# alexandrainst/coral

Hardware: AMD Instinct MI355X
Metric: audio-seconds/sec (CTC finetune step: fwd+bwd+allreduce+clip+AdamW), wav2vec2-large, 10 s utterances (higher is better)
Workload: dtype bf16; 1 GPU; wav2vec2-large (XLS-R shape d=1920 L=48 ffn=7680) CTC finetune, 8 x 10 s per GPU, SpecAugment on, activation_dropout 0.1, layerdrop 0 (multi-GPU rule), fp32 master + AdamW + clip 1.0; global_batch=8, frames_per_utt=499, parallelism=dp1

## Files before the change

### coral_amd/_lib.py

```python

from __future__ import annotations

import ctypes as C
import os
from pathlib import Path

_HERE = Path(__file__).resolve().parent
LIB_PATH = _HERE / "libcoral_amd.so"


class CoralAmdError(RuntimeError):
    """Raised when the HIP library is missing or a call into it fails."""


class CaGemmDesc(C.Structure):

    _fields_ = [
        ("A", C.c_void_p),
        ("B", C.c_void_p),
        ("C", C.c_void_p),
        ("C2", C.c_void_p),
        ("R", C.c_void_p),
        ("bias", C.c_void_p),
        ("M", C.c_int32),
# ... 220 lines not shown
                               _vp]),
    "ca_beam_select_workspace_bytes": (_i64, [_i32, _i32, _i32]),
    "ca_beam_select": (C.c_int, [_vp, _i64, _vp, _vp, _i32, _i32, _i32, _vp, _vp, _vp, _vp, _i64, _vp]),
    "ca_beam_advance": (C.c_int, [C.POINTER(CaBeamDesc), _vp]),
    "ca_mask_frames": (C.c_int, [_vp, _vp, _vp, _vp, _vp, _i32, _i32, _i32, _vp]),
    "ca_regroup_pad": (C.c_int, [_vp, _vp, _i32, _i32, _i32, _i32, _i32, _vp]),
    "ca_posconv_partial_floats": (_i64, [_i32]),
    "ca_posconv_weight": (C.c_int, [_vp, _vp, _vp, _vp, _vp, _vp, _i32, _i32, _i32, _vp]),
    "ca_posconv_weight_bwd": (
        C.c_int,
        [_vp, _vp, _vp, _vp, _vp, _vp, _vp, _i32, _i32, _i32, _vp],
    ),
    "ca_cast_f32_bf16": (C.c_int, [_vp, _vp, _i64, _vp]),
    "ca_cast_bf16_f32": (C.c_int, [_vp, _vp, _i64, _vp]),
    "ca_transpose_f32_bf16": (C.c_int, [_vp, _vp, _i32, _i32, _vp]),
    "ca_conv_weight_reorder": (C.c_int, [_vp, _vp, _i32, _i32, _i32, _vp]),
    "ca_conv_weight_grad_reorder": (C.c_int, [_vp, _vp, _i32, _i32, _i32, _vp]),
    "ca_sumsq_f32": (C.c_int, [_vp, _i64, _vp, _i32, _vp, _vp]),
    "ca_sumsq_ranges_f32": (C.c_int, [_vp, _vp, _i32, _vp, _i32, _vp, _vp]),
    "ca_clear_ranges": (C.c_int, [_vp, _vp, _i32, _i64, _vp]),
    "ca_sum_f32": (C.c_int, [_vp, _i64, _vp, _i32, _vp, _vp]),
    "ca_adamw_step": (
        C.c_int,
        [_vp, _vp, _vp, _vp, _vp, _i64, _f32, _f32, _f32, _f32, _f32, _i32, _f32, _f32, _vp, _vp],
    ),
    "ca_adamw_step_ex": (
        C.c_int,
        [_vp, _vp, _vp, _vp, _vp, _i64, _f32, _f32, _f32, _f32, _f32, _i32, _f32, _f32, _vp, _i32, _vp],
    ),
    "ca_adamw_step_g16": (
        C.c_int,
        [_vp, _vp, _vp, _vp, _vp, _i64, _f32, _f32, _f32, _f32, _f32, _i32, _f32, _f32, _vp, _i32, _vp],
    ),
    "ca_logmel_workspace_bytes": (_i64, [_i32]),
    "ca_logmel": (C.c_int, [_vp, _vp, _vp, _vp, _i32, _i64, _i32, _vp]),
    "ca_cross_entropy_fwd_bwd": (
        C.c_int,
        [_vp, _vp, _vp, _vp, _vp, _i64, _i32, _i64, _i32, _vp],
    ),
    "ca_argmax_masked": (C.c_int, [_vp, _vp, _vp, _i64, _i32, _i64, _vp]),
    "ca_whisper_decode_token": (C.c_int, [C.POINTER(CaDecodeDesc), _vp]),
    "ca_whisper_decode_token_supported": (C.c_int, [_i32, _i32, _i32, _i32, _i32]),
    "ca_debug_decode_stamps": (C.c_int, [_vp, _i32]),
    "ca_argmax_advance": (C.c_int, [_vp, _vp, _vp, _i64, _i32, _i64, _vp, _vp, _i64, _vp, _vp, _vp, _i32, _i32, _vp]),
    "ca_argmax_timestamps": (C.c_int, [_vp, _vp, _vp, _i64, _i32, _i64, _vp, _i64, _vp, _i32, _i32, _i32, _i32, _vp]),
    "ca_argmax_timestamps_advance": (C.c_int, [_vp, _vp, _vp, _i64, _i32, _i64, _vp, _vp, _i64, _vp, _vp, _vp, _i32, _i32,
                                               _i32, _i32, _i32, _vp]),
    "ca_pick_scored_advance": (C.c_int, [_vp, _vp, _vp, _i64, _i32, _i64, _f32, _vp, _i64, _vp, _vp, _vp, _vp, _i64, _vp, _vp,
                                         _vp, _i32, _i32, _vp, _i32, _i32, _i32, _vp]),
    "ca_row_token_prob": (C.c_int, [_vp, _vp, _i64, _i32, _i64, _i32, _vp]),
    "ca_whisper_align_cost": (C.c_int, [_vp, C.POINTER(_vp), _i32, C.POINTER(_i32), _i32, _i32, _i32, _i32, _i32, _i32, _i64,
                                        _i64, _vp, _i32, _f32, _i32, _vp, _vp, _i64, _vp]),
    "ca_dtw_token_times": (C.c_int, [_vp, _i32, _i32, _vp, _i32, _vp, _vp, _vp, _vp, _vp, _vp]),
    "ca_embed_tokens": (C.c_int, [_vp, _vp, _vp, _vp, _vp, _i64, _i32, _vp]),
    "ca_embed_tokens_bwd": (C.c_int, [_vp, _vp, _vp, _vp, _vp, _i64, _i32, _vp]),
    "ca_comm_unique_id": (C.c_int, [_vp]),
    "ca_comm_init": (C.c_int, [C.POINTER(_vp), _vp, _i32, _i32]),
    "ca_comm_destroy": (C.c_int, [_vp]),
    "ca_comm_abort": (C.c_int, [_vp]),
    "ca_comm_stream": (_vp, [_vp]),
    "ca_comm_rank": (C.c_int, [_vp]),
    "ca_comm_world": (C.c_int, [_vp]),
    "ca_comm_after": (C.c_int, [_vp, _vp]),
    "ca_comm_before": (C.c_int, [_vp, _vp]),
    "ca_allreduce_bucket": (C.c_int, [_vp, _vp, _i64, _i32]),
    "ca_reduce_scatter_bucket": (C.c_int, [_vp, _vp, _i64, _i32]),
# ... 30 lines not shown
```

### coral_amd/csrc/misc.hip

```cpp
#include "common.h"
#include <cstdlib>

__global__ __launch_bounds__(256) void mask_frames_kernel(unsigned short* __restrict__ h,
                                                          const uint8_t* __restrict__ tmask,
                                                          const uint8_t* __restrict__ fmask,
                                                          const unsigned short* __restrict__ embed,
                                                          const int32_t* __restrict__ flen, int B,
                                                          int T, int C) {
  const int cch = C >> 3;
  const int64_t total = (int64_t)B * T * cch;
  for (int64_t i = (int64_t)blockIdx.x * 256 + threadIdx.x; i < total;
       i += (int64_t)gridDim.x * 256) {
    const int c8 = (int)(i % cch);
    const int64_t bt = i / cch;
    const int t = (int)(bt % T), b = (int)(bt / T);
    const bool tm = tmask && tmask[bt];
    const bool pad = flen && t >= flen[b];
    bool anyf = false;
    if (fmask) {
#pragma unroll
      for (int e = 0; e < 8; ++e) anyf |= fmask[(int64_t)b * C + c8 * 8 + e] != 0;
    }
    if (!tm && !pad && !anyf) continue;
    unsigned short* p = h + bt * C + c8 * 8;
// ... 472 lines not shown
    if (threadIdx.x == 0) partial[c] = red[0] + red[1] + red[2] + red[3];
  }
}
extern "C" int ca_sumsq_ranges_f32(const float* g, const int64_t* chunks, int32_t nchunks, float* out,
                                   int32_t accumulate, float* partial, void* stream) {
  CA_CHECK_ARG(g && chunks && out && partial && nchunks > 0, "ca_sumsq_ranges_f32: bad argument");
  CA_CHECK_ARG(((uintptr_t)g % 16) == 0, "ca_sumsq_ranges_f32: g must be 16-byte aligned");
  hipStream_t s = (hipStream_t)stream;
  const int grid = nchunks < 2048 ? nchunks : 2048;
  hipLaunchKernelGGL(sumsq_chunks_kernel, dim3(grid), dim3(256), 0, s, g, chunks, nchunks, partial);
  hipLaunchKernelGGL(sumsq_finish_kernel, dim3(1), dim3(256), 0, s, partial, nchunks, out, accumulate);
  CA_CHECK_LAUNCH("ca_sumsq_ranges_f32");
  return CA_OK;
}
__global__ __launch_bounds__(256) void sum_kernel(const float* __restrict__ x, int64_t n, float* __restrict__ partial) {
  __shared__ float red[4];
  float a = 0.f;
  for (int64_t i = (int64_t)blockIdx.x * 256 + threadIdx.x; i < n; i += (int64_t)gridDim.x * 256) a += x[i];
  a = wave_sum(a);
  if ((threadIdx.x & 63) == 0) red[threadIdx.x >> 6] = a;
  __syncthreads();
  if (threadIdx.x == 0) partial[blockIdx.x] = red[0] + red[1] + red[2] + red[3];
}
extern "C" int ca_sum_f32(const float* x, int64_t n, float* out, int32_t accumulate, float* partial, void* stream) {
  CA_CHECK_ARG(x && out && partial && n > 0, "ca_sum_f32: bad argument");
  hipStream_t s = (hipStream_t)stream;
  const int grid = (int)((n + 255) / 256 < 256 ? (n + 255) / 256 : 256);
  hipLaunchKernelGGL(sum_kernel, dim3(grid), dim3(256), 0, s, x, n, partial);
  hipLaunchKernelGGL(sumsq_finish_kernel, dim3(1), dim3(256), 0, s, partial, grid, out, accumulate);
  CA_CHECK_LAUNCH("ca_sum_f32");
  return CA_OK;
}

template <bool NT, bool G16 = false>
__global__ __launch_bounds__(256) void adamw_kernel(float* __restrict__ p, float* __restrict__ m,
                                                    float* __restrict__ v,
                                                    const void* __restrict__ gv,
                                                    unsigned short* __restrict__ p16, int64_t n,
                                                    float lr, float b1, float b2, float eps,
                                                    float wd, float bc1, float bc2_sqrt,
                                                    float grad_scale, float max_norm,
                                                    const float* __restrict__ gnorm_sq, int allow_vec) {
  float coef = grad_scale;
  if (gnorm_sq && max_norm > 0.f) {
    const float nrm = sqrtf(gnorm_sq[0]) * grad_scale;
    const float c = max_norm / (nrm + 1e-6f);
    coef *= c < 1.f ? c : 1.f;
  }
  const float step_size = lr / bc1;
  const float decay = 1.f - lr * wd;
  const float* g = (const float*)gv;
  const unsigned short* g16 = (const unsigned short*)gv;
  const bool vec = allow_vec && ((((uintptr_t)p | (uintptr_t)m | (uintptr_t)v | (G16 ? 0 : (uintptr_t)gv)) & 15) == 0) &&
                   (!G16 || ((uintptr_t)gv & 7) == 0) && (!p16 || ((uintptr_t)p16 & 7) == 0);
  const int64_t n4 = vec ? (n >> 2) : 0;
  for (int64_t i = (int64_t)blockIdx.x * 256 + threadIdx.x; i < n4; i += (int64_t)gridDim.x * 256) {
    f32x4_t g4;
    if constexpr (G16) {
      const u16x4_t h = NT ? __builtin_nontemporal_load((const u16x4_t*)g16 + i) : ((const u16x4_t*)g16)[i];
      g4 = (f32x4_t){bf2f(h[0]), bf2f(h[1]), bf2f(h[2]), bf2f(h[3])};
    } else {
      g4 = NT ? __builtin_nontemporal_load((const f32x4_t*)g + i) : ((const f32x4_t*)g)[i];
    }
    f32x4_t p4 = NT ? __builtin_nontemporal_load((const f32x4_t*)p + i) : ((const f32x4_t*)p)[i];
    f32x4_t m4 = NT ? __builtin_nontemporal_load((const f32x4_t*)m + i) : ((const f32x4_t*)m)[i];
    f32x4_t v4 = NT ? __builtin_nontemporal_load((const f32x4_t*)v + i) : ((const f32x4_t*)v)[i];
    u16x4_t h4;
#pragma unroll
    for (int e = 0; e < 4; ++e) {
      const float gi = g4[e] * coef;
      float pi = p4[e] * decay;
      const float mi = b1 * m4[e] + (1.f - b1) * gi;
      const float vi = b2 * v4[e] + (1.f - b2) * gi * gi;
      const float denom = sqrtf(vi) / bc2_sqrt + eps;
      pi -= step_size * mi / denom;
      p4[e] = pi;
      m4[e] = mi;
      v4[e] = vi;
      h4[e] = f2bf(pi);
    }
    if (NT) {
      __builtin_nontemporal_store(p4, (f32x4_t*)p + i);
      __builtin_nontemporal_store(m4, (f32x4_t*)m + i);
      __builtin_nontemporal_store(v4, (f32x4_t*)v + i);
    } else {
      ((f32x4_t*)p)[i] = p4;
      ((f32x4_t*)m)[i] = m4;
      ((f32x4_t*)v)[i] = v4;
    }
    if (p16) ((u16x4_t*)p16)[i] = h4;
  }
  for (int64_t i = n4 * 4 + (int64_t)blockIdx.x * 256 + threadIdx.x; i < n; i += (int64_t)gridDim.x * 256) {
    const float gi = (G16 ? bf2f(g16[i]) : g[i]) * coef;
    float pi = p[i] * decay;
    const float mi = b1 * m[i] + (1.f - b1) * gi;
    const float vi = b2 * v[i] + (1.f - b2) * gi * gi;
    const float denom = sqrtf(vi) / bc2_sqrt + eps;
    pi -= step_size * mi / denom;
    p[i] = pi;
    m[i] = mi;
    v[i] = vi;
    if (p16) p16[i] = f2bf(pi);
  }
}
static int adamw_launch(float* p, float* m, float* v, const void* g, bool g16, void* p16, int64_t n, float lr, float beta1,
                        float beta2, float eps, float weight_decay, int32_t step, float grad_scale, float max_norm,
                        const float* gnorm_sq, int32_t max_blocks, void* stream) {
  CA_CHECK_ARG(p && m && v && g && n > 0 && step >= 1 && max_blocks >= 0, "ca_adamw_step: bad argument");
  const float bc1 = 1.f - powf(beta1, (float)step);
  const float bc2 = 1.f - powf(beta2, (float)step);
  static const int cap_env = [] { const char* e = getenv("CA_ADAMW_BLOCKS"); return e ? atoi(e) : 0; }();
  static const int vec = [] { const char* e = getenv("CA_ADAMW_VEC"); return e ? atoi(e) : 1; }();
  static const int nt = [] { const char* e = getenv("CA_ADAMW_NT"); return e ? atoi(e) : 1; }();
  const int cap = cap_env > 0 ? cap_env : max_blocks;
  int grid = ew_grid(n, vec ? 4 : 1);
  if (cap > 0 && grid > cap) grid = cap;
#define ADAMW(NTV, G16V)                                                                                              \
  hipLaunchKernelGGL((adamw_kernel<NTV, G16V>), dim3(grid), dim3(256), 0, (hipStream_t)stream, p, m, v, g,            \
                     (unsigned short*)p16, n, lr, beta1, beta2, eps, weight_decay, bc1, sqrtf(bc2), grad_scale,       \
                     max_norm, gnorm_sq, vec)
  if (nt && g16) ADAMW(true, true);
  else if (nt) ADAMW(true, false);
  else if (g16) ADAMW(false, true);
  else ADAMW(false, false);
#undef ADAMW
  CA_CHECK_LAUNCH("ca_adamw_step");
  return CA_OK;
}
const void* ca_adamw_background_kernel() { return (const void*)adamw_kernel<true, true>; }
extern "C" int ca_adamw_step_ex(float* p, float* m, float* v, const float* g, void* p16, int64_t n,
                                float lr, float beta1, float beta2, float eps, float weight_decay,
                                int32_t step, float grad_scale, float max_norm,
                                const float* gnorm_sq, int32_t max_blocks, void* stream) {
  return adamw_launch(p, m, v, g, false, p16, n, lr, beta1, beta2, eps, weight_decay, step, grad_scale, max_norm, gnorm_sq,
                      max_blocks, stream);
}
extern "C" int ca_adamw_step_g16(float* p, float* m, float* v, const void* g_bf16, void* p16, int64_t n,
                                 float lr, float beta1, float beta2, float eps, float weight_decay,
                                 int32_t step, float grad_scale, float max_norm,
                                 const float* gnorm_sq, int32_t max_blocks, void* stream) {
  return adamw_launch(p, m, v, g_bf16, true, p16, n, lr, beta1, beta2, eps, weight_decay, step, grad_scale, max_norm,
                      gnorm_sq, max_blocks, stream);
}
extern "C" int ca_adamw_step(float* p, float* m, float* v, const float* g, void* p16, int64_t n,
                             float lr, float beta1, float beta2, float eps, float weight_decay,
                             int32_t step, float grad_scale, float max_norm,
                             const float* gnorm_sq, void* stream) {
  return ca_adamw_step_ex(p, m, v, g, p16, n, lr, beta1, beta2, eps, weight_decay, step, grad_scale, max_norm, gnorm_sq, 0,
                          stream);
}

__global__ __launch_bounds__(256) void embed_kernel(const unsigned short* __restrict__ table,
                                                    const unsigned short* __restrict__ pos,
                                                    const int32_t* __restrict__ ids,
                                                    const int32_t* __restrict__ pos_ids,
                                                    unsigned short* __restrict__ y, int64_t rows,
                                                    int C) {
  const int cch = C >> 3;
  const int64_t total = rows * cch;
  for (int64_t i = (int64_t)blockIdx.x * 256 + threadIdx.x; i < total;
       i += (int64_t)gridDim.x * 256) {
    const int c8 = (int)(i % cch);
// ... 56 lines not shown
```

### coral_amd/ops.py

```python

from __future__ import annotations

import ctypes as C
import os

import torch

from . import _lib
from ._lib import (CaAttnDesc, EPI_DGELU, EPI_GELU, EPI_GELU_RESIDUAL, EPI_NONE, EPI_RESIDUAL, KMAJOR,
                   MNMAJOR, CaGemmDesc, CoralAmdError, check)

__all__ = ["KMAJOR", "MNMAJOR", "EPI_NONE", "EPI_GELU", "EPI_RESIDUAL", "EPI_DGELU",
           "EPI_GELU_RESIDUAL", "CoralAmdError"]

_ELT = {torch.bfloat16: 2, torch.float32: 4, torch.int32: 4, torch.uint8: 1, torch.int64: 8, torch.int16: 2,
        torch.uint32: 4}


def _stream() -> int:
    return torch.cuda.current_stream().cuda_stream


def _p(t: torch.Tensor | None, off: int = 0) -> int | None:
    if t is None:
# ... 571 lines not shown
        if any(a % 4 or n % 4 for a, n in rows):
            raise CoralAmdError("clear_ranges: ranges must be multiples of 4 bytes")
        big = [r for r in rows if r[1] >= (1 << 20)]
        small = [r for r in rows if r[1] < (1 << 20)]
        ent = tuple((torch.tensor(part, dtype=torch.int64, device=x.device), len(part), max(n for _, n in part))
                    for part in (big, small) if part)
        _CLEAR_TABLES[key] = ent
    for table, count, longest in ent:
        check(lib().ca_clear_ranges(_p(x), _p(table), count, longest, _stream()), "ca_clear_ranges")


def sumsq(g, n, out, partial, accumulate=False):
    check(lib().ca_sumsq_f32(_p(g), n, _p(out), int(accumulate), _p(partial), _stream()),
          "ca_sumsq_f32")


def sumsq_ranges(g, chunks, nchunks, out, partial, accumulate=False):
    check(lib().ca_sumsq_ranges_f32(_p(g), _p(chunks), nchunks, _p(out), int(accumulate), _p(partial), _stream()),
          "ca_sumsq_ranges_f32")


def sum_f32(x, n, out, partial, accumulate=False):
    check(lib().ca_sum_f32(_p(x), n, _p(out), int(accumulate), _p(partial), _stream()), "ca_sum_f32")


def adamw_step(p, m, v, g, p16, n, lr, beta1, beta2, eps, weight_decay, step, grad_scale=1.0,
               max_norm=0.0, gnorm_sq=None, max_blocks=0):
    fn = lib().ca_adamw_step_g16 if g.dtype == torch.bfloat16 else lib().ca_adamw_step_ex
    check(fn(_p(p), _p(m), _p(v), _p(g), _p(p16), n, lr, beta1, beta2, eps,
             weight_decay, step, grad_scale, max_norm, _p(gnorm_sq), int(max_blocks), _stream()),
          "ca_adamw_step")


def logmel_workspace_bytes(B):
    return lib().ca_logmel_workspace_bytes(B)


def logmel(wave, mel_filters, out, ws, B, N, n_mels):
    check(lib().ca_logmel(_p(wave), _p(mel_filters), _p(out), _p(ws), B, N, n_mels, _stream()),
          "ca_logmel")


def cross_entropy_fwd_bwd(logits, labels, loss_sum, count, grad, rows, V, ldv, ignore_index=-100):
    check(lib().ca_cross_entropy_fwd_bwd(_p(logits), _p(labels), _p(loss_sum), _p(count), _p(grad),
                                         rows, V, ldv, ignore_index, _stream()),
          "ca_cross_entropy_fwd_bwd")


def argmax_masked(logits, suppress, out, rows, V, ldv):
    check(lib().ca_argmax_masked(_p(logits), _p(suppress), _p(out), rows, V, ldv, _stream()),
          "ca_argmax_masked")


def argmax_advance(logits, suppress, out, rows, V, ldv, done, ids, tok, pos, klen, pad_id, eos_id):
    if done.dtype != torch.bool or ids.dtype != torch.int64 or ids.dim() != 2 or ids.stride(1) != 1:
        raise CoralAmdError("argmax_advance: done must be bool, ids a row-major int64 matrix")
    check(lib().ca_argmax_advance(_p(logits), _p(suppress), _p(out), rows, V, ldv, done.data_ptr(), _p(ids), ids.stride(0),
                                  _p(tok), _p(pos), _p(klen), int(pad_id), int(eos_id), _stream()), "ca_argmax_advance")


def _cap(max_initial_timestamp_index):
    return -1 if max_initial_timestamp_index is None else int(max_initial_timestamp_index)


def argmax_timestamps(logits, suppress, out, rows, V, ldv, ids, pos, begin_index, timestamp_begin, eos_id,
                      max_initial_timestamp_index=None):
# ... 185 lines not shown
```

### coral_amd/trainer.py

```python

from __future__ import annotations

import logging
import math
import os
import warnings

import torch

from . import ops
from .exchange import GradSync, collectives_selfcheck


def cosine_lr(step: int, base_lr: float, warmup_steps: int, max_steps: int) -> float:
    if step < warmup_steps:
        return base_lr * step / max(1, warmup_steps)
    progress = (step - warmup_steps) / max(1, max_steps - warmup_steps)
    return base_lr * max(0.0, 0.5 * (1.0 + math.cos(math.pi * progress)))


def grad_accumulation_steps(total_batch_size: int, num_devices: int, per_device_batch_size: int) -> int:
    return max(1, total_batch_size // max(1, num_devices) // per_device_batch_size)


# ... 60 lines not shown
        self.grad_accum = grad_accum
        if accum_loss not in ("mean", "sum"):
            raise ValueError(f"accum_loss must be 'mean' or 'sum', not {accum_loss!r}")
        self.accum_loss = accum_loss
        self.opt_step = 0
        st = engine.store
        lo, hi = self.train_range = tuple(engine.trainable_range())
        whole = (lo, hi) == (0, st.numel)
        world = 1
        if torch.distributed.is_available() and torch.distributed.is_initialized():
            world = torch.distributed.get_world_size(process_group)
        zero_stage = int(os.environ.get("CA_ZERO_STAGE", zero_stage) or 0)
        shard = {}
        if zero_stage and (world > 1 or os.environ.get("CA_DP_FORCE", "0") == "1") and whole:
            shard = {n: r for n, r in engine.shard_ranges().items() if (r[1] - r[0]) % (8 * world) == 0 and r[1] > r[0]}
        self.sync = GradSync(st.g32, st.buckets, process_group, compress=compress_grads, shard=shard)
        self.zero = bool(shard) and self.sync.active
        if self.zero and world > 1 and st.p32.is_cuda and not collectives_selfcheck(st.device, process_group, self.sync.capi):
            logging.getLogger(__package__).warning("sharded optimiser: the collective self-check failed; using replicated DDP")
            self.sync.close(abort=True)
            self.sync = GradSync(st.g32, st.buckets, process_group, compress=compress_grads)
            self.zero = False
        self.world = self.sync.world
        self.dist = self.sync.active
        self._set_compute_cus = False
        if self.dist and st.p32.is_cuda:
            ncu = torch.cuda.get_device_properties(st.device).multi_processor_count
            ops.lib().ca_gemm_set_compute_cus(int(os.environ.get("CA_COMPUTE_CUS", ncu)))
            self._set_compute_cus = True
        self.overlap = overlap and self.dist
        self._layout = state_layout(st.buckets, self.sync.shard if self.zero else {}, self.sync.rank, self.world)
        self._launches = [split_bf16(self._layout, r) for r in ({}, {} if self.zero else engine.bf16_grad_ranges())]
        self._forward_order = sorted(st.buckets, key=lambda name: st.buckets[name][0])
        self.m = torch.zeros(state_size(self._layout), dtype=torch.float32, device=st.device)
        self.v = torch.zeros_like(self.m)
        self._ag_comm = self.sync.capi if self.zero else None
        self._ag_stream = None
        if self.zero and st.p32.is_cuda:
            self._ag_stream = self._ag_comm.stream if self._ag_comm is not None else ops.side_stream(st.device, "gather")
        self.gnorm_sq = torch.zeros(1, dtype=torch.float32, device=st.device)
        self.partial = torch.zeros(4096, dtype=torch.float32, device=st.device)
        self.overlap_optimizer = (overlap_optimizer and os.environ.get("CA_OPT_OVERLAP", "1") != "0"
                                  and st.p32.is_cuda and whole)
        self.opt_stream = None
        if self.overlap_optimizer:
            prio = int(os.environ.get("CA_OPT_PRIO", "0"))
            self.opt_stream = ops.side_stream(st.device, "optimizer", prio)
        self.opt_done = None
        self.bg_blocks = 0
        if self.overlap_optimizer:
            bg = os.environ.get("CA_OPT_BG_BLOCKS")
            self.bg_blocks = int(bg) if bg is not None else torch.cuda.get_device_properties(st.device).multi_processor_count
            if bg is None:
                fits, rx, ru = ops.background_update_fits()
                if not fits:
                    warnings.warn(f"coral_amd: the forward GEMM kernel holds {rx} registers per lane and the update "
                                  f"kernel {ru}: the update cannot run beside it; using the full-grid update")
                    self.bg_blocks = 0
        self.bucket_index = {name: i for i, name in enumerate(st.buckets)}
        self.bucket_sq = torch.zeros(len(st.buckets), dtype=torch.float32, device=st.device)
        self.shard_norm = os.environ.get("CA_SHARD_NORM", "1") != "0"
        self._route = None
        self.partial_early = torch.zeros(4096, dtype=torch.float32, device=st.device)
        self.early_fraction = float(os.environ.get("CA_EARLY_NORM", "0.8"))
        self._early_lo = None
        self._done = {}
# ... 114 lines not shown
            torch.cuda.current_stream().wait_event(self.opt_done)
            self.opt_done = None

    def close(self):
        self.finish()
        if torch.cuda.is_available() and self.engine.store.p32.is_cuda:
            torch.cuda.synchronize()
        self._ag_comm = None
        self.sync.close()
        if self._set_compute_cus:
            ops.lib().ca_gemm_set_compute_cus(0)
            self._set_compute_cus = False

    def optimizer_step(self):
        eng, st = self.engine, self.engine.store
        lo, hi = self.train_range
        lr = cosine_lr(self.opt_step, self.lr, self.warmup_steps, self.max_steps)
        self.last_lr = lr
        self.opt_step += 1
        route, self._route = self._route or self._norm_route(last=False)[0], None
        self._finish_norm(route)
        max_blocks = self.bg_blocks if eng.background_optimizer else 0

        def adam(a, b, so, g):
            ops.adamw_step(st.p32[a:b], self.m[so:so + b - a], self.v[so:so + b - a], g[a:b], st.p16[a:b], b - a,
                           lr, self.betas[0], self.betas[1], self.eps, self.wd, self.opt_step,
                           grad_scale=1.0 / self.world, max_norm=self.max_grad_norm, gnorm_sq=self.gnorm_sq,
                           max_blocks=max_blocks)

        bf16 = bool(eng.matrix_grads_bf16 and eng.wgrad_bf16)

        def update(name):
            for a, b, so, half in self._launches[bf16][name]:
                adam(a, b, so, st.g16 if half else st.g32)
            if not self.zero or name not in self.sync.shard:
                return None
            self._ag_stream.wait_stream(torch.cuda.current_stream())
            with torch.cuda.stream(self._ag_stream):
                self._allgather_bf16(*self.sync.shard[name], *self.sync.slice_of(name))
            return self._ag_stream

        if not self.overlap_optimizer:
            if self.zero or bf16:
                for name in st.buckets:
                    update(name)
                if self.zero:
                    torch.cuda.current_stream().wait_stream(self._ag_stream)
            else:
                adam(lo, hi, lo, st.g32)
            if not eng.freeze_base:
                eng.refresh_derived()
            if eng.bucket_copies:
                for name in st.buckets:
                    eng.refresh_bucket(name)
            return
        self.opt_stream.wait_stream(torch.cuda.current_stream())
        events = {}
        with torch.cuda.stream(self.opt_stream):
            for name in self._forward_order:
                gathered_on = update(name)
                if eng.bucket_copies:
                    if gathered_on is not None:
                        self.opt_stream.wait_stream(gathered_on)
                    eng.refresh_bucket(name)
                parts = eng.derived_parts if name == "front" else ()
                if name == "front":
                    eng.refresh_derived(parts[0] if parts else None)
                ev = torch.cuda.Event()
                ev.record(gathered_on if (gathered_on is not None and not eng.bucket_copies) else self.opt_stream)
                events[name] = ev
                for part in parts[1:]:
                    eng.refresh_derived(part)
                    ev = torch.cuda.Event()
                    ev.record(self.opt_stream)
                    events[f"front_{part}"] = ev
            if "front" not in events:
                eng.refresh_derived()
            if eng.preclear_small_grads and not eng.freeze_base:
                eng.clear_small_grads()
                eng.pre_zeroed = True
            if self.zero:
                self.opt_stream.wait_stream(self._ag_stream)
            self.opt_done = torch.cuda.Event()
            self.opt_done.record(self.opt_stream)
        eng.weights_ready = events

    def _allgather_bf16(self, mlo, hi, a, b):
        p16, pg = self.engine.store.p16, self.sync.pg
        if self._ag_comm is not None:
            self._ag_comm.all_gather(p16[mlo:hi])
            return
        if self.sync._has_rs:
# ... 32 lines not shown
```

### include/coral_amd.h

```cpp
#ifndef CORAL_AMD_H
#define CORAL_AMD_H

#include <stdint.h>

#ifdef __cplusplus
extern "C" {
#endif

#define CA_OK 0
#define CA_ERR_ARG (-1)
#define CA_ERR_LAUNCH (-2)
#define CA_ERR_UNSUPPORTED (-3)

int ca_version(void);
const char* ca_last_error(void);
int ca_device_count(void);

#define CA_KMAJOR 0
#define CA_MNMAJOR 1

#define CA_EPI_NONE 0
#define CA_EPI_GELU 1
#define CA_EPI_RESIDUAL 2
#define CA_EPI_DGELU 3
// ... 266 lines not shown
                          int32_t Cg, int32_t K, void* stream);

int ca_pack_rows(const void* x, void* y, const int32_t* row_off, int32_t B, int32_t T, int32_t C, int32_t elt_bytes,
                 void* stream);
int ca_unpack_rows(const void* x, void* y, const int32_t* row_off, int32_t B, int32_t T, int32_t C, int32_t elt_bytes,
                   void* stream);

int ca_cast_f32_bf16(const float* x, void* y, int64_t n, void* stream);
int ca_cast_bf16_f32(const void* x, float* y, int64_t n, void* stream);
int ca_transpose_f32_bf16(const float* x, void* y, int32_t rows, int32_t cols, void* stream);
int ca_conv_weight_reorder(const float* w, void* wr, int32_t Co, int32_t Ci, int32_t k,
                           void* stream);
int ca_conv_weight_grad_reorder(const float* dwr, float* dw, int32_t Co, int32_t Ci,
                                int32_t k, void* stream);

int ca_sumsq_f32(const float* g, int64_t n, float* out, int32_t accumulate, float* partial,
                 void* stream);
int ca_clear_ranges(void* base, const int64_t* ranges_bytes, int32_t nranges, int64_t max_bytes, void* stream);
int ca_sumsq_ranges_f32(const float* g, const int64_t* chunks, int32_t nchunks, float* out, int32_t accumulate,
                        float* partial, void* stream);
int ca_sum_f32(const float* x, int64_t n, float* out, int32_t accumulate, float* partial, void* stream);
int ca_adamw_step(float* p, float* m, float* v, const float* g, void* p16, int64_t n,
                  float lr, float beta1, float beta2, float eps, float weight_decay,
                  int32_t step, float grad_scale, float max_norm, const float* gnorm_sq,
                  void* stream);
int ca_adamw_step_ex(float* p, float* m, float* v, const float* g, void* p16, int64_t n,
                     float lr, float beta1, float beta2, float eps, float weight_decay,
                     int32_t step, float grad_scale, float max_norm, const float* gnorm_sq,
                     int32_t max_blocks, void* stream);
int ca_adamw_step_g16(float* p, float* m, float* v, const void* g_bf16, void* p16, int64_t n,
                      float lr, float beta1, float beta2, float eps, float weight_decay,
                      int32_t step, float grad_scale, float max_norm, const float* gnorm_sq,
                      int32_t max_blocks, void* stream);
int ca_background_update_fits(int32_t* regs);

int64_t ca_logmel_workspace_bytes(int32_t B);
int ca_logmel(const float* wave, const float* mel_filters, float* out, void* ws, int32_t B,
              int64_t N, int32_t n_mels, void* stream);

int ca_cross_entropy_fwd_bwd(const float* logits, const int32_t* labels, float* loss_sum,
                             int32_t* count, float* grad, int64_t rows, int32_t V,
                             int64_t ldv, int32_t ignore_index, void* stream);
int ca_argmax_masked(const float* logits, const uint8_t* suppress, int32_t* out,
                     int64_t rows, int32_t V, int64_t ldv, void* stream);
int ca_argmax_advance(const float* logits, const uint8_t* suppress, int32_t* out, int64_t rows, int32_t V, int64_t ldv,
                      uint8_t* done, int64_t* ids, int64_t ld_ids, int32_t* tok, int32_t* pos, int32_t* klen,
                      int32_t pad_id, int32_t eos_id, void* stream);
int ca_argmax_timestamps(const float* logits, const uint8_t* suppress, int32_t* out, int64_t rows, int32_t V, int64_t ldv,
                         const int64_t* ids, int64_t ld_ids, const int32_t* pos, int32_t begin_index,
                         int32_t timestamp_begin, int32_t eos_id, int32_t max_initial_timestamp_index, void* stream);
int ca_argmax_timestamps_advance(const float* logits, const uint8_t* suppress, int32_t* out, int64_t rows, int32_t V,
                                 int64_t ldv, uint8_t* done, int64_t* ids, int64_t ld_ids, int32_t* tok, int32_t* pos,
                                 int32_t* klen, int32_t pad_id, int32_t eos_id, int32_t begin_index,
                                 int32_t timestamp_begin, int32_t max_initial_timestamp_index, void* stream);
int ca_pick_scored_advance(const float* logits, const uint8_t* suppress, int32_t* out, int64_t rows, int32_t V, int64_t ldv,
                           float inv_temperature, const float* uniforms, int64_t ld_u, float* sum_logprob,
                           int32_t* n_scored, uint8_t* done, int64_t* ids, int64_t ld_ids, int32_t* tok, int32_t* pos,
                           int32_t* klen, int32_t pad_id, int32_t eos_id, const int64_t* history, int32_t begin_index,
                           int32_t timestamp_begin, int32_t max_initial_timestamp_index, void* stream);
int ca_row_token_prob(const float* logits, float* out, int64_t rows, int32_t V, int64_t ldv, int32_t token, void* stream);
int ca_embed_tokens(const void* table, const void* pos, const int32_t* ids,
                    const int32_t* pos_ids, void* y, int64_t rows, int32_t C, void* stream);
int ca_embed_tokens_bwd(const void* dy, const int32_t* ids, const int32_t* pos_ids, float* dtable,
                        float* dpos, int64_t rows, int32_t C, void* stream);

#define CA_ALIGN_MAX_TOKENS 447
// ... 81 lines not shown
```

Before: 1144 audio-seconds/sec.

## Batch small fp32 AdamW ranges into one multi-range launch and add wide kernel

Measured after the change: 1143 audio-seconds/sec. No clear change (-0.1%).

```diff
diff --git a/coral_amd/_lib.py b/coral_amd/_lib.py
--- a/coral_amd/_lib.py
+++ b/coral_amd/_lib.py
@@ -276,6 +276,11 @@
         C.c_int,
         [_vp, _vp, _vp, _vp, _vp, _i64, _f32, _f32, _f32, _f32, _f32, _i32, _f32, _f32, _vp, _i32, _vp],
     ),
+    "ca_adamw_step_ranges": (
+        C.c_int,
+        [_vp, _vp, _vp, _vp, _vp, _vp, _i32, _i64, _f32, _f32, _f32, _f32, _f32, _i32, _f32, _f32, _vp, _i32, _vp],
+    ),
+    "ca_adamw_force_vec": (C.c_int, [C.c_int]),
     "ca_logmel_workspace_bytes": (_i64, [_i32]),
     "ca_logmel": (C.c_int, [_vp, _vp, _vp, _vp, _i32, _i64, _i32, _vp]),
     "ca_cross_entropy_fwd_bwd": (
diff --git a/coral_amd/csrc/misc.hip b/coral_amd/csrc/misc.hip
--- a/coral_amd/csrc/misc.hip
+++ b/coral_amd/csrc/misc.hip
@@ -528,76 +528,177 @@
   return CA_OK;
 }
 
-template <bool NT, bool G16 = false>
-__global__ __launch_bounds__(256) void adamw_kernel(float* __restrict__ p, float* __restrict__ m,
-                                                    float* __restrict__ v,
-                                                    const void* __restrict__ gv,
-                                                    unsigned short* __restrict__ p16, int64_t n,
-                                                    float lr, float b1, float b2, float eps,
-                                                    float wd, float bc1, float bc2_sqrt,
-                                                    float grad_scale, float max_norm,
-                                                    const float* __restrict__ gnorm_sq, int allow_vec) {
+struct AdamwCoef {
+  float coef, step_size, decay, b1, b2, eps, bc2_sqrt;
+};
+__device__ __forceinline__ AdamwCoef adamw_coef(float lr, float b1, float b2, float eps, float wd, float bc1, float bc2_sqrt,
+                                                float grad_scale, float max_norm, const float* __restrict__ gnorm_sq) {
   float coef = grad_scale;
   if (gnorm_sq && max_norm > 0.f) {
     const float nrm = sqrtf(gnorm_sq[0]) * grad_scale;
     const float c = max_norm / (nrm + 1e-6f);
     coef *= c < 1.f ? c : 1.f;
   }
-  const float step_size = lr / bc1;
-  const float decay = 1.f - lr * wd;
+  return AdamwCoef{coef, lr / bc1, 1.f - lr * wd, b1, b2, eps, bc2_sqrt};
+}
+__device__ __forceinline__ void adamw_elem(const AdamwCoef& k, float g, float& p, float& m, float& v) {
+#pragma clang fp contract(off)
+  const float gi = g * k.coef;
+  const float mi = __builtin_fmaf(1.f - k.b1, gi, k.b1 * m);
+  const float vi = __builtin_fmaf(k.b2, v, gi * ((1.f - k.b2) * gi));
+  const float denom = sqrtf(vi) / k.bc2_sqrt + k.eps;
+  p = __builtin_fmaf(p, k.decay, -(k.step_size * mi / denom));
+  m = mi;
+  v = vi;
+}
+__device__ __forceinline__ u16x4_t adamw_elem4(const AdamwCoef& k, const f32x4_t& g, f32x4_t& p, f32x4_t& m, f32x4_t& v) {
+  u16x4_t h;
+#pragma unroll
+  for (int e = 0; e < 4; ++e) {
+    float pi = p[e], mi = m[e], vi = v[e];
+    adamw_elem(k, g[e], pi, mi, vi);
+    p[e] = pi;
+    m[e] = mi;
+    v[e] = vi;
+    h[e] = f2bf(pi);
+  }
+  return h;
+}
+template <bool NT, typename T>
+__device__ __forceinline__ T adamw_ld(const T* a) {
+  return NT ? __builtin_nontemporal_load(a) : *a;
+}
+template <bool NT, typename T>
+__device__ __forceinline__ void adamw_st(T x, T* a) {
+  if (NT) __builtin_nontemporal_store(x, a);
+  else *a = x;
+}
+template <bool NT, bool G16>
+__device__ __forceinline__ void adamw_groups4(const AdamwCoef& k, float* __restrict__ p, float* __restrict__ m,
+                                              float* __restrict__ v, const void* __restrict__ gv,
+                                              unsigned short* __restrict__ p16, int64_t n4, int64_t first, int64_t stride) {
+  for (int64_t i = first; i < n4; i += stride) {
+    f32x4_t g4;
+    if constexpr (G16) {
+      const u16x4_t h = adamw_ld<NT>((const u16x4_t*)gv + i);
+      g4 = (f32x4_t){bf2f(h[0]), bf2f(h[1]), bf2f(h[2]), bf2f(h[3])};
+    } else {
+      g4 = adamw_ld<NT>((const f32x4_t*)gv + i);
+    }
+    f32x4_t p4 = adamw_ld<NT>((const f32x4_t*)p + i);
+    f32x4_t m4 = adamw_ld<NT>((const f32x4_t*)m + i);
+    f32x4_t v4 = adamw_ld<NT>((const f32x4_t*)v + i);
+    const u16x4_t h4 = adamw_elem4(k, g4, p4, m4, v4);
+    adamw_st<NT>(p4, (f32x4_t*)p + i);
+    adamw_st<NT>(m4, (f32x4_t*)m + i);
+    adamw_st<NT>(v4, (f32x4_t*)v + i);
+    if (p16) ((u16x4_t*)p16)[i] = h4;
+  }
+}
+template <bool NT, bool G16>
+__device__ __forceinline__ void adamw_groups8(const AdamwCoef& k, float* __restrict__ p, float* __restrict__ m,
+                                              float* __restrict__ v, const void* __restrict__ gv,
+                                              unsigned short* __restrict__ p16, int64_t n8, int64_t blk, int64_t nblk) {
+  for (int64_t c = blk * 256; c < n8; c += nblk * 256) {
+    if (c + threadIdx.x >= n8) break;
+    const unsigned i = threadIdx.x;
+    const f32x4_t *pp = (const f32x4_t*)(p + c * 8), *mp = (const f32x4_t*)(m + c * 8), *vp = (const f32x4_t*)(v + c * 8);
+    f32x4_t ga, gb;
+    if constexpr (G16) {
+      const u16x8_t h = adamw_ld<NT>((const u16x8_t*)gv + c + i);
+      ga = (f32x4_t){bf2f(h[0]), bf2f(h[1]), bf2f(h[2]), bf2f(h[3])};
+      gb = (f32x4_t){bf2f(h[4]), bf2f(h[5]), bf2f(h[6]), bf2f(h[7])};
+    } else {
+      ga = adamw_ld<NT>((const f32x4_t*)gv + c * 2 + 2 * i);
+      gb = adamw_ld<NT>((const f32x4_t*)gv + c * 2 + 2 * i + 1);
+    }
+    f32x4_t pa = adamw_ld<NT>(pp + 2 * i), pb = adamw_ld<NT>(pp + 2 * i + 1);
+    f32x4_t ma = adamw_ld<NT>(mp + 2 * i), mb = adamw_ld<NT>(mp + 2 * i + 1);
+    f32x4_t va = adamw_ld<NT>(vp + 2 * i), vb = adamw_ld<NT>(vp + 2 * i + 1);
+    __builtin_amdgcn_sched_barrier(0);
+    const u16x4_t ha = adamw_elem4(k, ga, pa, ma, va), hb = adamw_elem4(k, gb, pb, mb, vb);
+    const u16x8_t h8 = {ha[0], ha[1], ha[2], ha[3], hb[0], hb[1], hb[2], hb[3]};
+    adamw_st<NT>(pa, (f32x4_t*)pp + 2 * i);
+    adamw_st<NT>(pb, (f32x4_t*)pp + 2 * i + 1);
+    adamw_st<NT>(ma, (f32x4_t*)mp + 2 * i);
+    adamw_st<NT>(mb, (f32x4_t*)mp + 2 * i + 1);
+    adamw_st<NT>(va, (f32x4_t*)vp + 2 * i);
+    adamw_st<NT>(vb, (f32x4_t*)vp + 2 * i + 1);
+    if (p16) ((u16x8_t*)p16)[c + i] = h8;
+  }
+}
+template <bool NT, bool G16, int W>
+__device__ __forceinline__ void adamw_range(const AdamwCoef& k, float* __restrict__ p, float* __restrict__ m,
+                                            float* __restrict__ v, const void* __restrict__ gv,
+                                            unsigned short* __restrict__ p16, int64_t n, int allow_vec, int64_t blk,
+                                            int64_t nblk) {
   const float* g = (const float*)gv;
   const unsigned short* g16 = (const unsigned short*)gv;
-  const bool vec = allow_vec && ((((uintptr_t)p | (uintptr_t)m | (uintptr_t)v | (G16 ? 0 : (uintptr_t)gv)) & 15) == 0) &&
-                   (!G16 || ((uintptr_t)gv & 7) == 0) && (!p16 || ((uintptr_t)p16 & 7) == 0);
-  const int64_t n4 = vec ? (n >> 2) : 0;
-  for (int64_t i = (int64_t)blockIdx.x * 256 + threadIdx.x; i < n4; i += (int64_t)gridDim.x * 256) {
-    f32x4_t g4;
-    if constexpr (G16) {
-      const u16x4_t h = NT ? __builtin_nontemporal_load((const u16x4_t*)g16 + i) : ((const u16x4_t*)g16)[i];
-      g4 = (f32x4_t){bf2f(h[0]), bf2f(h[1]), bf2f(h[2]), bf2f(h[3])};
-    } else {
-      g4 = NT ? __builtin_nontemporal_load((const f32x4_t*)g + i) : ((const f32x4_t*)g)[i];
-    }
-    f32x4_t p4 = NT ? __builtin_nontemporal_load((const f32x4_t*)p + i) : ((const f32x4_t*)p)[i];
-    f32x4_t m4 = NT ? __builtin_nontemporal_load((const f32x4_t*)m + i) : ((const f32x4_t*)m)[i];
-    f32x4_t v4 = NT ? __builtin_nontemporal_load((const f32x4_t*)v + i) : ((const f32x4_t*)v)[i];
-    u16x4_t h4;
-#pragma unroll
-    for (int e = 0; e < 4; ++e) {
-      const float gi = g4[e] * coef;
-      float pi = p4[e] * decay;
-      const float mi = b1 * m4[e] + (1.f - b1) * gi;
-      const float vi = b2 * v4[e] + (1.f - b2) * gi * gi;
-      const float denom = sqrtf(vi) / bc2_sqrt + eps;
-      pi -= step_size * mi / denom;
-      p4[e] = pi;
-      m4[e] = mi;
-      v4[e] = vi;
-      h4[e] = f2bf(pi);
-    }
-    if (NT) {
-      __builtin_nontemporal_store(p4, (f32x4_t*)p + i);
-      __builtin_nontemporal_store(m4, (f32x4_t*)m + i);
-      __builtin_nontemporal_store(v4, (f32x4_t*)v + i);
-    } else {
-      ((f32x4_t*)p)[i] = p4;
-      ((f32x4_t*)m)[i] = m4;
-      ((f32x4_t*)v)[i] = v4;
-    }
-    if (p16) ((u16x4_t*)p16)[i] = h4;
-  }
-  for (int64_t i = n4 * 4 + (int64_t)blockIdx.x * 256 + threadIdx.x; i < n; i += (int64_t)gridDim.x * 256) {
-    const float gi = (G16 ? bf2f(g16[i]) : g[i]) * coef;
-    float pi = p[i] * decay;
-    const float mi = b1 * m[i] + (1.f - b1) * gi;
-    const float vi = b2 * v[i] + (1.f - b2) * gi * gi;
-    const float denom = sqrtf(vi) / bc2_sqrt + eps;
-    pi -= step_size * mi / denom;
+  const uintptr_t a32 = (uintptr_t)p | (uintptr_t)m | (uintptr_t)v | (G16 ? 0 : (uintptr_t)gv);
+  const uintptr_t a16 = (G16 ? (uintptr_t)gv : 0) | (uintptr_t)p16;
+  const bool vec = allow_vec && (a32 & 15) == 0 && (a16 & 7) == 0;
+  const int64_t first = blk * 256 + threadIdx.x, stride = nblk * 256;
+  int64_t done = 0;
+  if constexpr (W == 8) {
+    if (vec && (a16 & 15) == 0) {
+      adamw_groups8<NT, G16>(k, p, m, v, gv, p16, n >> 3, blk, nblk);
+      done = (n >> 3) << 3;
+    }
+  }
+  if (vec) {
+    const int64_t n4 = (n - done) >> 2;
+    adamw_groups4<NT, G16>(k, p + done, m + done, v + done, G16 ? (const void*)(g16 + done) : (const void*)(g + done),
+                           p16 ? p16 + done : nullptr, n4, first, stride);
+    done += n4 << 2;
+  }
+  for (int64_t i = done + first; i < n; i += stride) {
+    float pi = p[i], mi = m[i], vi = v[i];
+    adamw_elem(k, G16 ? bf2f(g16[i]) : g[i], pi, mi, vi);
     p[i] = pi;
     m[i] = mi;
     v[i] = vi;
     if (p16) p16[i] = f2bf(pi);
   }
+}
+#define ADAMW_PARAMS                                                                                                   \
+  float *__restrict__ p, float *__restrict__ m, float *__restrict__ v, const void *__restrict__ gv,                    \
+      unsigned short *__restrict__ p16, int64_t n, float lr, float b1, float b2, float eps, float wd, float bc1,      \
+      float bc2_sqrt, float grad_scale, float max_norm, const float *__restrict__ gnorm_sq, int allow_vec
+template <bool NT, bool G16 = false>
+__global__ __launch_bounds__(256) void adamw_kernel(ADAMW_PARAMS) {
+  const AdamwCoef k = adamw_coef(lr, b1, b2, eps, wd, bc1, bc2_sqrt, grad_scale, max_norm, gnorm_sq);
+  adamw_range<NT, G16, 4>(k, p, m, v, gv, p16, n, allow_vec, blockIdx.x, gridDim.x);
+}
+template <bool NT, bool G16 = false>
+__global__ __launch_bounds__(256) void adamw_wide_kernel(ADAMW_PARAMS) {
+  const AdamwCoef k = adamw_coef(lr, b1, b2, eps, wd, bc1, bc2_sqrt, grad_scale, max_norm, gnorm_sq);
+  adamw_range<NT, G16, 8>(k, p, m, v, gv, p16, n, allow_vec, blockIdx.x, gridDim.x);
+}
+#undef ADAMW_PARAMS
+template <bool NT>
+__global__ __launch_bounds__(256) void adamw_ranges_kernel(float* __restrict__ p, float* __restrict__ m,
+                                                           float* __restrict__ v, const float* __restrict__ g,
+                                                           unsigned short* __restrict__ p16,
+                                                           const int64_t* __restrict__ ranges, int nranges, float lr,
+                                                           float b1, float b2, float eps, float wd, float bc1,
+                                                           float bc2_sqrt, float grad_scale, float max_norm,
+                                                           const float* __restrict__ gnorm_sq, int allow_vec) {
+  const AdamwCoef k = adamw_coef(lr, b1, b2, eps, wd, bc1, bc2_sqrt, grad_scale, max_norm, gnorm_sq);
+  for (int r = blockIdx.y; r < nranges; r += gridDim.y) {
+    const int64_t off = ranges[3 * r], n = ranges[3 * r + 1], so = ranges[3 * r + 2];
+    adamw_range<NT, false, 4>(k, p + off, m + so, v + so, g + off, p16 ? p16 + off : nullptr, n, allow_vec, blockIdx.x,
+                              gridDim.x);
+  }
+}
+#define CA_ADAMW_VEC_DEFAULT 1
+static int g_adamw_vec = -1;
+static int adamw_vec() {
+  static const int vec = [] { const char* e = getenv("CA_ADAMW_VEC"); return e ? atoi(e) : CA_ADAMW_VEC_DEFAULT; }();
+  return g_adamw_vec >= 0 ? g_adamw_vec : vec;
+}
+extern "C" int ca_adamw_force_vec(int vec) {
+  g_adamw_vec = vec;
+  return CA_OK;
 }
 static int adamw_launch(float* p, float* m, float* v, const void* g, bool g16, void* p16, int64_t n, float lr, float beta1,
                         float beta2, float eps, float weight_decay, int32_t step, float grad_scale, float max_norm,
@@ -606,24 +707,56 @@
   const float bc1 = 1.f - powf(beta1, (float)step);
   const float bc2 = 1.f - powf(beta2, (float)step);
   static const int cap_env = [] { const char* e = getenv("CA_ADAMW_BLOCKS"); return e ? atoi(e) : 0; }();
-  static const int vec = [] { const char* e = getenv("CA_ADAMW_VEC"); return e ? atoi(e) : 1; }();
   static const int nt = [] { const char* e = getenv("CA_ADAMW_NT"); return e ? atoi(e) : 1; }();
+  const int vec = adamw_vec();
   const int cap = cap_env > 0 ? cap_env : max_blocks;
-  int grid = ew_grid(n, vec ? 4 : 1);
+  int grid = ew_grid(n, vec >= 2 ? 8 : vec ? 4 : 1);
   if (cap > 0 && grid > cap) grid = cap;
-#define ADAMW(NTV, G16V)                                                                                              \
-  hipLaunchKernelGGL((adamw_kernel<NTV, G16V>), dim3(grid), dim3(256), 0, (hipStream_t)stream, p, m, v, g,            \
+#define ADAMW(KERNEL, NTV, G16V)                                                                                      \
+  hipLaunchKernelGGL((KERNEL<NTV, G16V>), dim3(grid), dim3(256), 0, (hipStream_t)stream, p, m, v, g,                  \
                      (unsigned short*)p16, n, lr, beta1, beta2, eps, weight_decay, bc1, sqrtf(bc2), grad_scale,       \
                      max_norm, gnorm_sq, vec)
-  if (nt && g16) ADAMW(true, true);
-  else if (nt) ADAMW(true, false);
-  else if (g16) ADAMW(false, true);
-  else ADAMW(false, false);
+#define ADAMW_FORM(KERNEL)                                                                                            \
+  do {                                                                                                                \
+    if (nt && g16) ADAMW(KERNEL, true, true);                                                                         \
+    else if (nt) ADAMW(KERNEL, true, false);                                                                          \
+    else if (g16) ADAMW(KERNEL, false, true);                                                                         \
+    else ADAMW(KERNEL, false, false);                                                                                 \
+  } while (0)
+  if (vec >= 2) ADAMW_FORM(adamw_wide_kernel);
+  else ADAMW_FORM(adamw_kernel);
+#undef ADAMW_FORM
 #undef ADAMW
   CA_CHECK_LAUNCH("ca_adamw_step");
   return CA_OK;
 }
-const void* ca_adamw_background_kernel() { return (const void*)adamw_kernel<true, true>; }
+const void* ca_adamw_background_kernel() {
+  return adamw_vec() >= 2 ? (const void*)adamw_wide_kernel<true, true> : (const void*)adamw_kernel<true, true>;
+}
+extern "C" int ca_adamw_step_ranges(float* p, float* m, float* v, const float* g, void* p16, const int64_t* ranges,
+                                    int32_t nranges, int64_t max_len, float lr, float beta1, float beta2, float eps,
+                                    float weight_decay, int32_t step, float grad_scale, float max_norm,
+                                    const float* gnorm_sq, int32_t max_blocks, void* stream) {
+  CA_CHECK_ARG(p && m && v && g && ranges && nranges > 0 && max_len > 0 && step >= 1 && max_blocks >= 0,
+               "ca_adamw_step_ranges: bad argument");
+  const float bc1 = 1.f - powf(beta1, (float)step);
+  const float bc2 = 1.f - powf(beta2, (float)step);
+  static const int nt = [] { const char* e = getenv("CA_ADAMW_NT"); return e ? atoi(e) : 1; }();
+  const int vec = adamw_vec();
+  const int gy = nranges < 1024 ? nranges : 1024;
+  int gx = ew_grid(max_len, vec ? 4 : 1);
+  if (gx > 64) gx = 64;
+  if (max_blocks > 0 && gx * gy > max_blocks) gx = max_blocks / gy > 0 ? max_blocks / gy : 1;
+#define ADAMW(NTV)                                                                                                     \
+  hipLaunchKernelGGL((adamw_ranges_kernel<NTV>), dim3(gx, gy), dim3(256), 0, (hipStream_t)stream, p, m, v, g,          \
+                     (unsigned short*)p16, ranges, nranges, lr, beta1, beta2, eps, weight_decay, bc1, sqrtf(bc2),      \
+                     grad_scale, max_norm, gnorm_sq, vec)
+  if (nt) ADAMW(true);
+  else ADAMW(false);
+#undef ADAMW
+  CA_CHECK_LAUNCH("ca_adamw_step_ranges");
+  return CA_OK;
+}
 extern "C" int ca_adamw_step_ex(float* p, float* m, float* v, const float* g, void* p16, int64_t n,
                                 float lr, float beta1, float beta2, float eps, float weight_decay,
                                 int32_t step, float grad_scale, float max_norm,
diff --git a/coral_amd/ops.py b/coral_amd/ops.py
--- a/coral_amd/ops.py
+++ b/coral_amd/ops.py
@@ -627,6 +627,16 @@
           "ca_adamw_step")
 
 
+def adamw_step_ranges(p, m, v, g, p16, ranges, nranges, max_len, lr, beta1, beta2, eps, weight_decay, step,
+                      grad_scale=1.0, max_norm=0.0, gnorm_sq=None, max_blocks=0):
+    if g.dtype != torch.float32 or ranges.dtype != torch.int64 or not ranges.is_contiguous():
+        raise CoralAmdError("adamw_step_ranges: fp32 gradients and a contiguous int64 range table")
+    check(lib().ca_adamw_step_ranges(_p(p), _p(m), _p(v), _p(g), _p(p16), _p(ranges), int(nranges), int(max_len), lr,
+                                     beta1, beta2, eps, weight_decay, step, grad_scale, max_norm, _p(gnorm_sq),
+                                     int(max_blocks), _stream()),
+          "ca_adamw_step_ranges")
+
+
 def logmel_workspace_bytes(B):
     return lib().ca_logmel_workspace_bytes(B)
 
diff --git a/coral_amd/trainer.py b/coral_amd/trainer.py
--- a/coral_amd/trainer.py
+++ b/coral_amd/trainer.py
@@ -116,6 +116,12 @@
         self._layout = state_layout(st.buckets, self.sync.shard if self.zero else {}, self.sync.rank, self.world)
         self._launches = [split_bf16(self._layout, r) for r in ({}, {} if self.zero else engine.bf16_grad_ranges())]
         self._forward_order = sorted(st.buckets, key=lambda name: st.buckets[name][0])
+        self._small = None
+        small = [(a, b - a, so) for segs in self._launches[1].values() if any(seg[3] for seg in segs)
+                 for a, b, so, inside in segs if not inside]
+        if small and st.p32.is_cuda and os.environ.get("CA_OPT_SMALL_RANGES", "1") != "0":
+            self._small = (torch.tensor(small, dtype=torch.int64, device=st.device), len(small), max(n for _, n, _ in small),
+                           {name for name, segs in self._launches[1].items() if any(seg[3] for seg in segs)})
         self.m = torch.zeros(state_size(self._layout), dtype=torch.float32, device=st.device)
         self.v = torch.zeros_like(self.m)
         self._ag_comm = self.sync.capi if self.zero else None
@@ -296,7 +302,8 @@
 
         def update(name):
             for a, b, so, half in self._launches[bf16][name]:
-                adam(a, b, so, st.g16 if half else st.g32)
+                if half or not (small and name in small[3]):
+                    adam(a, b, so, st.g16 if half else st.g32)
             if not self.zero or name not in self.sync.shard:
                 return None
             self._ag_stream.wait_stream(torch.cuda.current_stream())
@@ -304,6 +311,7 @@
                 self._allgather_bf16(*self.sync.shard[name], *self.sync.slice_of(name))
             return self._ag_stream
 
+        small = self._small if bf16 and self.overlap_optimizer else None
         if not self.overlap_optimizer:
             if self.zero or bf16:
                 for name in st.buckets:
@@ -321,7 +329,14 @@
         self.opt_stream.wait_stream(torch.cuda.current_stream())
         events = {}
         with torch.cuda.stream(self.opt_stream):
+            small_due = small is not None
             for name in self._forward_order:
+                if small_due and name in small[3]:
+                    small_due = False
+                    ops.adamw_step_ranges(st.p32, self.m, self.v, st.g32, st.p16, small[0], small[1], small[2], lr,
+                                          self.betas[0], self.betas[1], self.eps, self.wd, self.opt_step,
+                                          grad_scale=1.0 / self.world, max_norm=self.max_grad_norm,
+                                          gnorm_sq=self.gnorm_sq, max_blocks=max_blocks)
                 gathered_on = update(name)
                 if eng.bucket_copies:
                     if gathered_on is not None:
diff --git a/include/coral_amd.h b/include/coral_amd.h
--- a/include/coral_amd.h
+++ b/include/coral_amd.h
@@ -322,6 +322,11 @@
                       float lr, float beta1, float beta2, float eps, float weight_decay,
                       int32_t step, float grad_scale, float max_norm, const float* gnorm_sq,
                       int32_t max_blocks, void* stream);
+int ca_adamw_step_ranges(float* p, float* m, float* v, const float* g, void* p16, const int64_t* ranges,
+                         int32_t nranges, int64_t max_len, float lr, float beta1, float beta2, float eps,
+                         float weight_decay, int32_t step, float grad_scale, float max_norm, const float* gnorm_sq,
+                         int32_t max_blocks, void* stream);
+int ca_adamw_force_vec(int vec);
 int ca_background_update_fits(int32_t* regs);
 
 int64_t ca_logmel_workspace_bytes(int32_t B);
```
